# jiangzhengkai/mxdetection

Measured on AMD Instinct MI355X. Metric: images/sec (whole node) Faster R-CNN R50-FPN 3x800x1333, higher is better.
Workload: dtype bf16; 1 GPU; Faster R-CNN ResNet-50-FPN bf16 train step, batch 2/GPU, 3x800x1333 (padded 1344); global_batch=2, parallelism=dp1, frozen=stem+C2, frozen BN folded, optimizer=SGD momentum 0.9 wd 1e-4, launch=hipGraph replay, input=resident, wgrad_side_stream=True, rpn_branch_stream=True, grouped_wgrad=True, filter_prefetch_hints=True, params_trainable=41538304

## Files before the change

### include/mxdet.h

```cpp
#ifndef MXDET_H_
#define MXDET_H_

#include <stddef.h>
#include <stdint.h>

#ifdef __cplusplus
extern "C" {
#endif

#define MXDET_OK 0
#define MXDET_EINVAL (-1)
#define MXDET_ESHAPE (-2)
#define MXDET_EWORKSPACE (-3)
#define MXDET_EHIP (-4)
#define MXDET_ERCCL (-5)

#define MXDET_DTYPE_F32 0
#define MXDET_DTYPE_BF16 1

typedef void* mxdet_stream_t;

const char* mxdet_last_error(void);
const char* mxdet_version(void);

// ... 241 lines not shown
} mxdet_wgrad_item_t;
size_t mxdet_conv2d_wgrad_grouped_table_bytes(int32_t n);
int mxdet_conv2d_wgrad_grouped_plan(const mxdet_wgrad_item_t* items, int32_t n, void* table_host, size_t table_bytes,
                                    size_t* workspace_bytes, int32_t* grid_wgrad, int32_t* grid_big,
                                    int32_t* grid_reduce);
int mxdet_conv2d_wgrad_grouped(const void* table_dev, int32_t n, int32_t grid_wgrad, int32_t grid_big,
                               int32_t grid_reduce, void* workspace, size_t workspace_bytes, size_t workspace_needed,
                               mxdet_stream_t stream);
int mxdet_conv2d_wgrad_grouped_parts(const void* table_dev, int32_t n, int32_t grid_wgrad, int32_t grid_big,
                                     int32_t grid_reduce, int32_t parts, void* workspace, size_t workspace_bytes,
                                     size_t workspace_needed, mxdet_stream_t stream);
int mxdet_filter_transpose(const uint16_t* w, int32_t Cout, int32_t KH, int32_t KW, int32_t Cin,
                           uint16_t* wt, mxdet_stream_t stream);

int mxdet_filter_transpose_batched(const void* descs_dev, int32_t ndesc, int32_t total_tiles,
                                   mxdet_stream_t stream);

#define MXDET_RPN_SPARSE_MAX_LEVELS 8
#define MXDET_RPN_SPARSE_ZERO 1
#define MXDET_RPN_SPARSE_DT 2
#define MXDET_RPN_SPARSE_WGRAD 4
#define MXDET_RPN_SPARSE_DGRAD 8
#define MXDET_RPN_SPARSE_DTMAP 16
typedef struct {
  int32_t num_levels, N, A, C, Ch, smax;
  int32_t H[MXDET_RPN_SPARSE_MAX_LEVELS], W[MXDET_RPN_SPARSE_MAX_LEVELS];
  int32_t accumulate[MXDET_RPN_SPARSE_MAX_LEVELS];
  const void* P[MXDET_RPN_SPARSE_MAX_LEVELS];
  const void* t[MXDET_RPN_SPARSE_MAX_LEVELS];
  const void* tbits[MXDET_RPN_SPARSE_MAX_LEVELS];
  const void* gh[MXDET_RPN_SPARSE_MAX_LEVELS];
  void* dP[MXDET_RPN_SPARSE_MAX_LEVELS];
  void* dt[MXDET_RPN_SPARSE_MAX_LEVELS];
} mxdet_rpn_sparse_t;
int mxdet_rpn_sparse_list(const mxdet_rpn_sparse_t* d, const int32_t* labels, int32_t* list, int32_t* state,
                          int32_t* map, mxdet_stream_t stream);
int mxdet_rpn_sparse_backward(const mxdet_rpn_sparse_t* d, const int32_t* list, const int32_t* state,
                              const int32_t* map, const uint16_t* wt_out, const uint16_t* wt_conv, uint16_t* dts,
                              uint16_t* ghs, float* dw_out, float* db_out, float* dw_conv, float* db_conv,
                              int32_t parts, mxdet_stream_t stream);

typedef struct {
  int32_t N, H, W, C;
  int32_t Ho, Wo;
  int32_t KH, KW;
  int32_t stride, pad;
  int32_t groups;
  int32_t modulated;
  int32_t off_channels;
  int32_t accumulate;
} mxdet_deform_desc_t;
int mxdet_deform_im2col(const mxdet_deform_desc_t* d, const uint16_t* x, const uint16_t* off, uint16_t* col,
                        mxdet_stream_t stream);
int mxdet_deform_col2im_coord(const mxdet_deform_desc_t* d, const uint16_t* x, const uint16_t* off,
                              const uint16_t* dcol, uint16_t* doff, mxdet_stream_t stream);
size_t mxdet_deform_col2im_workspace_bytes(const mxdet_deform_desc_t* d);
int mxdet_deform_col2im(const mxdet_deform_desc_t* d, const uint16_t* off, const uint16_t* dcol, uint16_t* dx,
                        void* workspace, size_t workspace_bytes, mxdet_stream_t stream);

typedef struct {
  int32_t N, HW, C, G;
  float eps;
  int32_t relu;
// ... 81 lines not shown
```

### mxdetection_amd/_lib.py

```python
import ctypes as C
import os

_HERE = os.path.dirname(os.path.abspath(__file__))
LIB_PATH = os.environ.get("MXDET_LIB") or os.path.join(_HERE, "libmxdet_hip.so")

c_i32, c_i64, c_u32, c_f32, c_sz, c_vp = C.c_int32, C.c_int64, C.c_uint32, C.c_float, C.c_size_t, C.c_void_p


class PyramidT(C.Structure):
    _fields_ = [
        ("num_levels", c_i32), ("A", c_i32),
        ("H", c_i32 * 8), ("W", c_i32 * 8), ("stride", c_i32 * 8),
        ("cls", c_vp * 8), ("reg", c_vp * 8),
        ("cls_sn", c_i64 * 8), ("cls_sy", c_i64 * 8), ("cls_sx", c_i64 * 8), ("cls_sa", c_i64 * 8),
        ("reg_sn", c_i64 * 8), ("reg_sy", c_i64 * 8), ("reg_sx", c_i64 * 8), ("reg_sc", c_i64 * 8),
        ("dtype", c_i32), ("classes", c_i32),
        ("base_anchors", c_vp * 8),
    ]


class FeatPyramidT(C.Structure):
    _fields_ = [
        ("num_levels", c_i32), ("lvl_min", c_i32),
        ("H", c_i32 * 8), ("W", c_i32 * 8),
# ... 28 lines not shown

class DeformDescT(C.Structure):
    _fields_ = [
        ("N", c_i32), ("H", c_i32), ("W", c_i32), ("C", c_i32),
        ("Ho", c_i32), ("Wo", c_i32), ("KH", c_i32), ("KW", c_i32),
        ("stride", c_i32), ("pad", c_i32), ("groups", c_i32), ("modulated", c_i32),
        ("off_channels", c_i32), ("accumulate", c_i32),
    ]


class DpoolDescT(C.Structure):
    _fields_ = [
        ("pyr", FeatPyramidT), ("N", c_i32), ("C", c_i32), ("PH", c_i32), ("PW", c_i32),
        ("sample_per_part", c_i32), ("trans_std", c_f32), ("modulated", c_i32),
        ("trans_stride", c_i32), ("mask_stride", c_i32), ("accumulate", c_i32),
    ]


class GnDescT(C.Structure):
    _fields_ = [("N", c_i32), ("HW", c_i32), ("C", c_i32), ("G", c_i32), ("eps", c_f32), ("relu", c_i32),
                ("accumulate", c_i32)]


class RpnSparseT(C.Structure):
    _fields_ = [("num_levels", c_i32), ("N", c_i32), ("A", c_i32), ("C", c_i32), ("Ch", c_i32), ("smax", c_i32),
                ("H", c_i32 * 8), ("W", c_i32 * 8), ("accumulate", c_i32 * 8),
                ("P", c_vp * 8), ("t", c_vp * 8), ("tbits", c_vp * 8), ("gh", c_vp * 8), ("dP", c_vp * 8), ("dt", c_vp * 8)]


WgradItemT._fields_ = [("desc", ConvDescT), ("x", c_vp), ("dy", c_vp), ("dw", c_vp), ("db", c_vp)]
ConvItemT._fields_ = [("desc", ConvDescT), ("src", c_vp), ("filt", c_vp), ("bias", c_vp), ("residual", c_vp),
                      ("relu_mask", c_vp), ("dst", c_vp)]

P = C.POINTER

SIGNATURES = {
    "mxdet_last_error": (C.c_char_p, []),
    "mxdet_version": (C.c_char_p, []),
    "mxdet_box_iou": (c_i32, [c_vp, c_i64, c_vp, c_i64, c_vp, c_vp]),
    "mxdet_generate_anchors": (c_i32, [c_vp, c_i32, c_i32, c_i32, c_i32, c_vp, c_vp]),
    "mxdet_nms_batched_workspace_bytes": (c_sz, [c_i32, c_i32]),
    "mxdet_nms_batched": (c_i32, [c_vp, c_vp, c_vp, c_i32, c_i32, c_f32, c_i32, c_vp, c_vp, c_vp, c_sz, c_vp]),
    "mxdet_soft_nms_batched": (c_i32, [c_vp, c_vp, c_vp, c_i32, c_i32, c_i32, c_f32, c_f32, c_f32, c_i32, c_vp, c_vp, c_vp,
                                       c_vp]),
    "mxdet_pixel_shuffle2_inv_relu": (c_i32, [c_vp, c_vp, c_i64, c_i32, c_i32, c_i32, c_vp, c_vp]),
    "mxdet_mask_paste_workspace_bytes": (c_sz, [c_i64, c_i32]),
    "mxdet_mask_paste": (c_i32, [c_vp, c_vp, c_i64, c_i32, c_i32, c_i32, c_i32, c_f32, c_vp, c_vp, c_sz, c_vp]),
    "mxdet_retina_detect_workspace_bytes": (c_sz, [c_vp, c_i32, c_i32]),
    "mxdet_retina_detect": (c_i32, [c_vp, c_i32, c_vp, c_i32, c_f32, c_f32, c_i32, c_vp, c_vp, c_vp, c_sz, c_vp]),
    "mxdet_retina_detect_soft": (c_i32, [c_vp, c_i32, c_vp, c_i32, c_f32, c_f32, c_i32, c_vp, c_vp, c_vp, c_sz, c_i32, c_f32,
# ... 58 lines not shown
    "mxdet_pixel_shuffle2": (c_i32, [c_vp, c_i64, c_i32, c_i32, c_i32, c_i32, c_vp, c_vp]),
    "mxdet_mask_loss_workspace_bytes": (c_sz, [c_i64, c_i32]),
    "mxdet_mask_loss": (c_i32, [c_vp, c_vp, c_vp, c_i64, c_i32, c_i32, c_f32, c_vp, c_vp, c_vp, c_sz, c_vp]),
    "mxdet_conv2d_fwd": (c_i32, [P(ConvDescT), c_vp, c_vp, c_vp, c_vp, c_vp, c_vp]),
    "mxdet_conv2d_fwd_chain": (c_i32, [P(ConvDescT), c_vp, c_vp, c_vp, c_vp, c_vp, c_i32, c_i32, c_vp, c_vp, c_vp, c_vp, c_i32,
                                       c_i32, c_vp, c_vp]),
    "mxdet_conv2d_fwd_splitk_workspace_bytes": (c_sz, [P(ConvDescT), c_i32]),
    "mxdet_conv2d_fwd_splitk": (c_i32, [P(ConvDescT), c_vp, c_vp, c_vp, c_vp, c_vp, c_i32, c_vp, c_sz, c_vp]),
    "mxdet_conv2d_dgrad": (c_i32, [P(ConvDescT), c_vp, c_vp, c_vp, c_vp, c_vp, c_vp]),
    "mxdet_conv2d_wgrad_workspace_bytes": (c_sz, [P(ConvDescT)]),
    "mxdet_conv2d_wgrad": (c_i32, [P(ConvDescT), c_vp, c_vp, c_vp, c_vp, c_vp, c_sz, c_vp]),
    "mxdet_conv2d_grouped_table_bytes": (c_sz, [c_i32]),
    "mxdet_conv2d_grouped_plan": (c_i32, [P(ConvItemT), c_i32, c_i32, c_vp, c_sz, P(c_i32), P(c_i32)]),
    "mxdet_conv2d_grouped": (c_i32, [c_vp, c_i32, c_i32, c_i32, c_i32, c_vp]),
    "mxdet_conv2d_wgrad_grouped_table_bytes": (c_sz, [c_i32]),
    "mxdet_conv2d_wgrad_grouped_plan": (c_i32, [P(WgradItemT), c_i32, c_vp, c_sz, P(c_sz), P(c_i32), P(c_i32), P(c_i32)]),
    "mxdet_conv2d_wgrad_grouped": (c_i32, [c_vp, c_i32, c_i32, c_i32, c_i32, c_vp, c_sz, c_sz, c_vp]),
    "mxdet_conv2d_wgrad_grouped_parts": (c_i32, [c_vp, c_i32, c_i32, c_i32, c_i32, c_i32, c_vp, c_sz, c_sz, c_vp]),
    "mxdet_debug_force_conv_cfg": (c_i32, [c_i32]),
    "mxdet_debug_force_wgrad_ksplit": (c_i32, [c_i32]),
    "mxdet_rpn_sparse_list": (c_i32, [P(RpnSparseT), c_vp, c_vp, c_vp, c_vp, c_vp]),
    "mxdet_rpn_sparse_backward": (c_i32, [P(RpnSparseT), c_vp, c_vp, c_vp, c_vp, c_vp, c_vp, c_vp, c_vp, c_vp, c_vp, c_vp,
                                          c_i32, c_vp]),
    "mxdet_filter_transpose": (c_i32, [c_vp, c_i32, c_i32, c_i32, c_i32, c_vp, c_vp]),
    "mxdet_filter_transpose_batched": (c_i32, [c_vp, c_i32, c_i32, c_vp]),
    "mxdet_deform_im2col": (c_i32, [P(DeformDescT), c_vp, c_vp, c_vp, c_vp]),
    "mxdet_deform_col2im_coord": (c_i32, [P(DeformDescT), c_vp, c_vp, c_vp, c_vp, c_vp]),
    "mxdet_deform_col2im_workspace_bytes": (c_sz, [P(DeformDescT)]),
    "mxdet_deform_col2im": (c_i32, [P(DeformDescT), c_vp, c_vp, c_vp, c_vp, c_sz, c_vp]),
    "mxdet_dpool_fwd": (c_i32, [P(DpoolDescT), c_vp, c_vp, c_i64, c_vp, c_vp, c_vp, c_vp]),
    "mxdet_dpool_bwd_trans": (c_i32, [P(DpoolDescT), c_vp, c_vp, c_i64, c_vp, c_vp, c_vp, c_vp, c_vp, c_vp]),
    "mxdet_dpool_bwd_feat_workspace_bytes": (c_sz, [P(DpoolDescT), c_i64]),
    "mxdet_dpool_bwd_feat": (c_i32, [P(DpoolDescT), c_vp, c_vp, c_i64, c_vp, c_vp, c_vp, c_vp, c_sz, c_vp]),
    "mxdet_group_norm_workspace_bytes": (c_sz, [P(GnDescT), c_i32]),
    "mxdet_group_norm_fwd": (c_i32, [P(GnDescT), c_vp, c_vp, c_vp, c_vp, c_vp, c_vp, c_vp, c_sz, c_vp]),
    "mxdet_group_norm_bwd": (c_i32, [P(GnDescT), c_vp, c_vp, c_vp, c_vp, c_vp, c_vp, c_vp, c_vp, c_vp, c_vp, c_vp, c_sz,
                                     c_vp]),
    "mxdet_debug_group_norm_route": (c_i32, [P(GnDescT)]),
    "mxdet_stem_conv7x7": (c_i32, [c_vp, c_i32, c_i32, c_i32, c_i32, c_vp, c_vp, c_vp, c_vp]),
    "mxdet_stem_conv7x7_pool": (c_i32, [c_vp, c_i32, c_i32, c_i32, c_i32, c_vp, c_vp, c_vp, c_vp]),
    "mxdet_maxpool3x3s2": (c_i32, [c_vp, c_i32, c_i32, c_i32, c_i32, c_vp, c_vp]),
    "mxdet_subsample2": (c_i32, [c_vp, c_i32, c_i32, c_i32, c_i32, c_vp, c_vp]),
    "mxdet_subsample2_bwd": (c_i32, [c_vp, c_i32, c_i32, c_i32, c_i32, c_i32, c_vp, c_vp]),
    "mxdet_upsample2_bwd": (c_i32, [c_vp, c_i32, c_i32, c_i32, c_i32, c_i32, c_vp, c_vp]),
    "mxdet_add_bf16": (c_i32, [c_vp, c_vp, c_i64, c_vp, c_vp]),
    "mxdet_relu_bwd_bf16": (c_i32, [c_vp, c_vp, c_i64, c_vp, c_vp]),
# ... 73 lines not shown
```

### mxdetection_amd/csrc/rpn_sparse.hip

```cpp
#include "common.h"

namespace mxdet {

constexpr int kSpLevels = MXDET_RPN_SPARSE_MAX_LEVELS;
constexpr int kSpMaxSlots = 8192;

struct SpGeo {
  int L, N, A, C, Ch, smax, CT;
  int H[kSpLevels], W[kSpLevels], coff[kSpLevels + 1];
  const uint16_t* P[kSpLevels];
  const uint16_t* t[kSpLevels];
  const unsigned char* tbits[kSpLevels];
  const uint16_t* gh[kSpLevels];
  uint16_t* dP[kSpLevels];
  uint16_t* dt[kSpLevels];
  int acc[kSpLevels];
  const int* list;
  const int* state;
  const int* map;
  const uint16_t* wt_out;
  const uint16_t* wt_conv;
  uint16_t* dts;
  uint16_t* ghs;
  float* dw_out;
// ... 240 lines not shown
            const bf16x8_t bw = *(const bf16x8_t*)(wbase + (size_t)j * 16 * K9 + t * g.C + k);
            acc[j] = __builtin_amdgcn_mfma_f32_16x16x32_bf16(a, bw, acc[j], 0, 0, 0);
          }
        }
      }
    }
#pragma unroll
    for (int r = 0; r < 4; ++r) {
      const int row = fq * 4 + r;
      const int rl = __shfl(dl, row), rpix = __shfl(dpix, row);
      if (rpix < 0) continue;
      uint16_t* drow = g.dP[rl] + (size_t)rpix * g.C + cit * 64 + frow;
      const bool accum = g.acc[rl] != 0;
#pragma unroll
      for (int j = 0; j < 4; ++j) {
        float v = acc[j][r] + 0.0f;
        if (accum) v += bf16_bits_to_f32(drow[j * 16]);
        drow[j * 16] = sp_bf16(v);
      }
    }
  }
}

static int sp_zero_levels(const SpGeo& g, uint16_t* const* ptr, const int* skip, hipStream_t s) {
  for (int l = 0; l < g.L;) {
    if (skip && skip[l]) { ++l; continue; }
    MXDET_REQUIRE(ptr[l] != nullptr && ((uintptr_t)ptr[l] & 15) == 0, MXDET_EINVAL, "rpn_sparse_backward: level %d null / unaligned", l);
    char* p0 = (char*)ptr[l];
    char* p1 = p0;
    while (l < g.L && !(skip && skip[l]) && (char*)ptr[l] == p1) {
      p1 += (size_t)g.N * g.H[l] * g.W[l] * g.C * 2;
      ++l;
    }
    const long long n16 = (long long)(p1 - p0) / 16;
    hipLaunchKernelGGL(rpn_sparse_zero_kernel, dim3((unsigned)ceil_div<long long>(n16, 256)), dim3(256), 0, s, (uint4*)p0, n16);
  }
  return MXDET_OK;
}

static int sp_fill(SpGeo& g, const mxdet_rpn_sparse_t* d, const char* who) {
  MXDET_REQUIRE(d != nullptr, MXDET_EINVAL, "%s: null descriptor", who);
  MXDET_REQUIRE(d->num_levels > 0 && d->num_levels <= kSpLevels && d->N > 0 && d->A > 0, MXDET_ESHAPE,
                "%s: 1..%d levels, N > 0, A > 0", who, kSpLevels);
  MXDET_REQUIRE(d->C > 0 && d->C % 64 == 0 && d->Ch == 64, MXDET_ESHAPE, "%s: C %d must be a multiple of 64 and Ch %d must be 64",
                who, d->C, d->Ch);
  MXDET_REQUIRE(d->smax > 0 && d->smax <= kSpMaxSlots, MXDET_ESHAPE, "%s: smax %d must be in 1..%d", who, d->smax, kSpMaxSlots);
// ... 57 lines not shown
    for (int l = 0; l < g.L; ++l) g.dt[l] = (uint16_t*)d->dt[l];
    rc = sp_zero_levels(g, g.dt, nullptr, s);
    if (rc) return rc;
  }
  if (parts & MXDET_RPN_SPARSE_DT) {
    MXDET_REQUIRE(wt_out, MXDET_EINVAL, "rpn_sparse_backward: null wt_out");
    for (int l = 0; l < g.L; ++l)
      MXDET_REQUIRE(g.gh[l] && (g.tbits[l] || g.t[l]), MXDET_EINVAL, "rpn_sparse_backward: level %d: null gh / mask", l);
    hipLaunchKernelGGL(rpn_sparse_dt_kernel, dim3((unsigned)ceil_div(g.smax, 16)), dim3(64), 0, s, g);
  }
  if (parts & MXDET_RPN_SPARSE_WGRAD) {
    MXDET_REQUIRE(dw_out && db_out && dw_conv && db_conv, MXDET_EINVAL, "rpn_sparse_backward: null weight-gradient pointer");
    for (int l = 0; l < g.L; ++l)
      MXDET_REQUIRE(g.P[l] && g.t[l], MXDET_EINVAL, "rpn_sparse_backward: level %d: null P / t", l);
    const int ct = g.C / 64;
    hipLaunchKernelGGL(rpn_sparse_wgrad_kernel, dim3((unsigned)(9 * ct * ct + ct)), dim3(256), 0, s, g);
  }
  if (parts & MXDET_RPN_SPARSE_DGRAD) {
    MXDET_REQUIRE(wt_conv, MXDET_EINVAL, "rpn_sparse_backward: null wt_conv");
    for (int l = 0; l < g.L; ++l)
      MXDET_REQUIRE(g.dP[l], MXDET_EINVAL, "rpn_sparse_backward: level %d: null dP", l);
    hipLaunchKernelGGL(rpn_sparse_dgrad_kernel, dim3((unsigned)ceil_div(9 * g.smax, 16)), dim3(256), 0, s, g);
  }
  return check_launch("rpn_sparse_backward");
}
```

### mxdetection_amd/models/rpn_heads/rpn_head.py

```python
import os

import torch

from ...core import anchor as A_
from ...core import loss as L_
from ...ops import dense
from ...ops.proposal import PyramidProposal
from ...ops import rpn_sparse as RS
from ...ops.rpn_sparse import MAX_SLOTS, RPNSparse
from ..utils.layers import ConvLayer, cached_buf

HEAD_CPAD = 64


RELU_BITS = os.environ.get("MXDET_TUNE_RELU_BITS", "1") == "1"
RPN_SPARSE = int(os.environ.get("MXDET_TUNE_RPN_SPARSE", "1"))


class RPNHead:
    def __init__(self, channels, strides, arena, ws, device, gen, ratios=(0.5, 1.0, 2.0), scales=(8,),
                 pre_nms_top_n=2000, post_nms_top_n=2000, nms_thresh=0.7, min_size=0.0, batch_size=256,
                 fg_fraction=0.5, fg_thresh=0.7, bg_thresh=0.3, sigma=3.0, seed=99):
        kw = dict(arena=arena, ws=ws, device=device, gen=gen)
        self.A = len(ratios) * len(scales)
        assert 5 * self.A <= HEAD_CPAD
        self.out = ConvLayer("rpn.out", channels, HEAD_CPAD, 1, init_std=0.01, cout_real=5 * self.A, **kw)
        self.conv = ConvLayer("rpn.conv", channels, channels, 3, init_std=0.01, **kw)
        self.strides = list(strides)
        self.base = [torch.from_numpy(A_.generate_base_anchors(s, ratios, scales)).to(device) for s in strides]
        self.proposal = PyramidProposal(self.base, strides, pre_nms_top_n, post_nms_top_n, nms_thresh, min_size)
        self.batch_size, self.fg_fraction, self.fg_thresh, self.bg_thresh = batch_size, fg_fraction, fg_thresh, bg_thresh
        self.sigma, self.seed, self.device, self.C = sigma, seed, device, channels
        self.bufs = {}
        self.anchors = None
        self.level_shapes = None

    def layers(self):
        return [self.out, self.conv]

# ... 83 lines not shown
        grouped = self.out.ws.grouping
        for l in range(L):
            self.out.backward_weight(self.t[l], self.gh[l], accumulate=(l > 0) and not grouped)
        self.out.backward_data(self.gh[0], self.t[0].shape, relu_mask=self.t[0], out=dt[0], relu_bits=self.tbits[0])
        dense.conv2d_group("dgrad", [self.out.dgrad_call(self.gh[l], self.t[l].shape, relu_mask=self.t[l], out=dt[l],
                                                         relu_bits=self.tbits[l])
                                     for l in range(1, L)], self.device)
        for l in range(L):
            self.conv.backward_weight(self.P[l], dt[l], accumulate=(l > 0) and not grouped)
        self.conv.backward_data(dt[0], self.P[0].shape, accumulate=dP_has_grad[0], out=dP[0])
        dense.conv2d_group("dgrad", [self.conv.dgrad_call(dt[l], self.P[l].shape, accumulate=dP_has_grad[l], out=dP[l])
                                     for l in range(1, L)], self.device)
        if flush:
            self.out.ws.flush()

    def _backward_sparse(self, dP, dP_has_grad, flush=True):
        g = self.out.arena
        grads = (g.view(self.out.wi, "g"), g.view(self.out.bi, "g"), g.view(self.conv.wi, "g"), g.view(self.conv.bi, "g"))
        if self.sparse_wgrad:
            self.sparse.backward(self.P, self.t, self.tbits, self.gh, dP, dP_has_grad, self.out.wt, self.conv.wt, *grads)
            return
        L = len(self.h)
        grouped = self.out.ws.grouping
        for l in range(L):
            self.out.backward_weight(self.t[l], self.gh[l], accumulate=(l > 0) and not grouped)
        self.sparse.backward(self.P, self.t, self.tbits, self.gh, dP, dP_has_grad, self.out.wt, self.conv.wt, *grads,
                             parts=RS.ZERO | RS.DT | RS.DTMAP | RS.DGRAD, dt=self.dt_map)
        for l in range(L):
            self.conv.backward_weight(self.P[l], self.dt_map[l], accumulate=(l > 0) and not grouped)
        if flush:
            self.out.ws.flush()
```

### mxdetection_amd/ops/dense.py

```python
import ctypes as C

import torch

from .. import _lib
from .._lib import ConvDescT, check, ptr, stream_ptr

_DT = {torch.float32: 0, torch.bfloat16: 1}


def mem_range(*tensors):
    spans = [(t.data_ptr(), t.numel() * t.element_size()) for t in tensors]
    bases = {t.untyped_storage().data_ptr() for t in tensors}
    if len(bases) == 1:
        lo = min(p for p, _ in spans)
        hi = max(p + n for p, n in spans)
        if hi - lo <= 2 * sum(n for _, n in set(spans)):
            return (lo, hi - lo)
    return spans[0]


def conv_desc(N, H, W, Cin, Cout, KH, KW, stride, pad, relu=False, res_upsample=False, accumulate=False, prefetch=None,
              relu_bits=None):
    d = ConvDescT()
    if relu_bits is not None:
# ... 140 lines not shown
    key = (kind,) + tuple(tuple(t.data_ptr() if torch.is_tensor(t) else t for t in c) for c in calls)
    if PF_TRACE is not None and calls:
        PF_TRACE.append((None, "g", mem_range(*[c[1] for c in calls]), key if len(calls) > 1 else None))
    if len(calls) == 1:
        plan = None
    else:
        plan = _group_plans.get(key)
        if plan is None and not torch.cuda.is_current_stream_capturing():
            plan = GroupedConv(kind, calls, device, GROUP_HINTS.get(key))
            _group_plans[key] = plan
    if plan is not None:
        plan.launch()
        return
    for c in calls:
        if kind == "fwd":
            x, w, bias, residual, stride, pad, relu, res_up, out = c[:9]
            conv2d_forward(x, w, bias, residual, stride, pad, relu, res_up, out, bits_out=c[9] if len(c) > 9 else None)
        else:
            dy, wt, x_shape, KH, KW, stride, pad, residual, relu_mask, accumulate, out = c[:11]
            conv2d_dgrad(dy, wt, x_shape, KH, KW, stride, pad, residual, relu_mask, accumulate, out,
                         relu_bits=c[11] if len(c) > 11 else None)


class GroupedWgrad:

    def __init__(self, calls, device):
        lib = _lib.load()
        n = len(calls)
        items = (_lib.WgradItemT * n)()
        self.keep = calls
        self.flops = 0.0
        self.heaviest = (0.0, "")
        for it, (x, dy, KH, KW, stride, pad, dw, db, accumulate) in zip(items, calls):
            N, H, W, Cin = x.shape
            it.desc = conv_desc(N, H, W, Cin, dy.shape[3], KH, KW, stride, pad, accumulate=accumulate)
            it.x, it.dy, it.dw, it.db = x.data_ptr(), dy.data_ptr(), dw.data_ptr(), (db.data_ptr() if db is not None else None)
            fl = 2.0 * dy.shape[0] * dy.shape[1] * dy.shape[2] * dy.shape[3] * KH * KW * Cin
            self.flops += fl
            if fl > self.heaviest[0]:
                self.heaviest = (fl, "N=%d %dx%d %d->%d %dx%d" % (N, H, W, Cin, dy.shape[3], KH, KW))
        nbytes = lib.mxdet_conv2d_wgrad_grouped_table_bytes(n)
        host = (C.c_ubyte * nbytes)()
        ws, gw, gb, gr = C.c_size_t(0), C.c_int32(0), C.c_int32(0), C.c_int32(0)
        check(lib.mxdet_conv2d_wgrad_grouped_plan(items, n, host, nbytes, C.byref(ws), C.byref(gw), C.byref(gb),
                                                  C.byref(gr)), "conv2d_wgrad_grouped_plan")
        self.grid_big = gb.value
        self.table = torch.frombuffer(bytearray(host), dtype=torch.uint8).clone().to(device)
        self.n, self.grid_wgrad, self.grid_reduce, self.workspace_bytes = n, gw.value, gr.value, ws.value

    def launch(self, workspace):
        check(_lib.load().mxdet_conv2d_wgrad_grouped(ptr(self.table), self.n, self.grid_wgrad, self.grid_big, self.grid_reduce,
                                                     ptr(workspace), workspace.numel() if workspace is not None else 0,
                                                     self.workspace_bytes, stream_ptr()), "conv2d_wgrad_grouped")


def filter_transpose(w, out=None):
    lib = _lib.load()
    Cout, KH, KW, Cin = w.shape
    if out is None:
        out = torch.empty((Cin, KH, KW, Cout), dtype=torch.bfloat16, device=w.device)
    check(lib.mxdet_filter_transpose(ptr(w), Cout, KH, KW, Cin, ptr(out), stream_ptr()), "filter_transpose")
    return out


def make_transpose_table(pairs, device):
    import struct
    buf = bytearray()
    tile0 = 0
    for w, wt in pairs:
        Cout, KH, KW, Cin = w.shape
        buf += struct.pack("<QQiiii", w.data_ptr(), wt.data_ptr(), Cout, KH * KW, Cin, tile0)
# ... 150 lines not shown
```

### mxdetection_amd/ops/rpn_sparse.py

```python
import ctypes as C

import torch

from .. import _lib
from .._lib import RpnSparseT, check, ptr, stream_ptr

ZERO, DT, WGRAD, DGRAD, DTMAP = 1, 2, 4, 8, 16
ALL = ZERO | DT | WGRAD | DGRAD
MAX_SLOTS = 8192


class RPNSparse:

    def __init__(self, level_shapes, N, A, C_, Ch, smax, device):
        self.level_shapes, self.N, self.A, self.C, self.Ch, self.smax = list(level_shapes), N, A, C_, Ch, smax
        self.CT = sum(h * w for h, w in level_shapes)
        i32 = dict(dtype=torch.int32, device=device)
        self.list = torch.full((2 * smax,), -1, **i32)
        self.state = torch.zeros((2,), **i32)
        self.map = torch.full((N * self.CT,), -1, **i32)
        self.dts = torch.zeros((smax, C_), dtype=torch.bfloat16, device=device)
        self.ghs = torch.zeros((smax, Ch), dtype=torch.bfloat16, device=device)
        self._descs = {}

    def _desc(self, P=None, t=None, tbits=None, gh=None, dP=None, accumulate=None, dt=None):
        L = len(self.level_shapes)
        ops = (P, t, tbits, gh, dP, dt)
        key = tuple(None if o is None else tuple(0 if x is None else x.data_ptr() for x in o) for o in ops)
        key += (None if accumulate is None else tuple(bool(a) for a in accumulate),)
        d = self._descs.get(key)
        if d is None:
            d = RpnSparseT()
            d.num_levels, d.N, d.A, d.C, d.Ch, d.smax = L, self.N, self.A, self.C, self.Ch, self.smax
            for l, (h, w) in enumerate(self.level_shapes):
                d.H[l], d.W[l] = h, w
                d.accumulate[l] = int(bool(accumulate[l])) if accumulate is not None else 0
                for name, o in zip(("P", "t", "tbits", "gh", "dP", "dt"), ops):
                    if o is not None and o[l] is not None:
                        getattr(d, name)[l] = o[l].data_ptr()
            self._descs[key] = d
        return d

    def build_list(self, labels):
        assert labels.dtype == torch.int32 and labels.numel() == self.N * self.CT * self.A and labels.is_contiguous()
        check(_lib.load().mxdet_rpn_sparse_list(C.byref(self._desc()), ptr(labels), ptr(self.list), ptr(self.state),
                                                ptr(self.map), stream_ptr()), "rpn_sparse_list")

    def backward(self, P, t, tbits, gh, dP, accumulate, wt_out, wt_conv, dw_out, db_out, dw_conv, db_conv, parts=ALL, dt=None):
        d = self._desc(P, t, tbits, gh, dP, accumulate, dt)
        check(_lib.load().mxdet_rpn_sparse_backward(C.byref(d), ptr(self.list), ptr(self.state), ptr(self.map), ptr(wt_out),
                                                    ptr(wt_conv), ptr(self.dts), ptr(self.ghs), ptr(dw_out), ptr(db_out),
                                                    ptr(dw_conv), ptr(db_conv), parts, stream_ptr()), "rpn_sparse_backward")
```

Before: 452.6 images/sec.

## Add ordered sparse RPN weight-gradient kernel replacing dense grouped wgrad for head

```diff
diff --git a/include/mxdet.h b/include/mxdet.h
--- a/include/mxdet.h
+++ b/include/mxdet.h
@@ -287,6 +287,17 @@
 #define MXDET_RPN_SPARSE_WGRAD 4
 #define MXDET_RPN_SPARSE_DGRAD 8
 #define MXDET_RPN_SPARSE_DTMAP 16
+#define MXDET_RPN_SPARSE_WGRAD_ORDERED 32
+#define MXDET_RPN_ORDERED_WORK_INTS(smax) (10 * (smax) + 32)
+typedef struct {
+  int32_t kind;
+  int32_t H, W;
+  int32_t halves_per_slab;
+  int32_t slab0;
+  int32_t fold_ksplit;
+  int32_t bias_pixels;
+  int32_t bias_splits;
+} mxdet_rpn_ordered_item_t;
 typedef struct {
   int32_t num_levels, N, A, C, Ch, smax;
   int32_t H[MXDET_RPN_SPARSE_MAX_LEVELS], W[MXDET_RPN_SPARSE_MAX_LEVELS];
@@ -297,6 +308,8 @@
   const void* gh[MXDET_RPN_SPARSE_MAX_LEVELS];
   void* dP[MXDET_RPN_SPARSE_MAX_LEVELS];
   void* dt[MXDET_RPN_SPARSE_MAX_LEVELS];
+  const mxdet_rpn_ordered_item_t* ordered;
+  void* ordered_work;
 } mxdet_rpn_sparse_t;
 int mxdet_rpn_sparse_list(const mxdet_rpn_sparse_t* d, const int32_t* labels, int32_t* list, int32_t* state,
                           int32_t* map, mxdet_stream_t stream);
@@ -304,6 +317,7 @@
                               const int32_t* map, const uint16_t* wt_out, const uint16_t* wt_conv, uint16_t* dts,
                               uint16_t* ghs, float* dw_out, float* db_out, float* dw_conv, float* db_conv,
                               int32_t parts, mxdet_stream_t stream);
+int mxdet_rpn_ordered_schedule(const void* table_host, int32_t n, int32_t num_levels, mxdet_rpn_ordered_item_t* items);
 
 typedef struct {
   int32_t N, H, W, C;
diff --git a/mxdetection_amd/_lib.py b/mxdetection_amd/_lib.py
--- a/mxdetection_amd/_lib.py
+++ b/mxdetection_amd/_lib.py
@@ -74,10 +74,16 @@
                 ("accumulate", c_i32)]
 
 
+class RpnOrderedItemT(C.Structure):
+    _fields_ = [("kind", c_i32), ("H", c_i32), ("W", c_i32), ("halves_per_slab", c_i32), ("slab0", c_i32),
+                ("fold_ksplit", c_i32), ("bias_pixels", c_i32), ("bias_splits", c_i32)]
+
+
 class RpnSparseT(C.Structure):
     _fields_ = [("num_levels", c_i32), ("N", c_i32), ("A", c_i32), ("C", c_i32), ("Ch", c_i32), ("smax", c_i32),
                 ("H", c_i32 * 8), ("W", c_i32 * 8), ("accumulate", c_i32 * 8),
-                ("P", c_vp * 8), ("t", c_vp * 8), ("tbits", c_vp * 8), ("gh", c_vp * 8), ("dP", c_vp * 8), ("dt", c_vp * 8)]
+                ("P", c_vp * 8), ("t", c_vp * 8), ("tbits", c_vp * 8), ("gh", c_vp * 8), ("dP", c_vp * 8), ("dt", c_vp * 8),
+                ("ordered", C.POINTER(RpnOrderedItemT)), ("ordered_work", c_vp)]
 
 
 WgradItemT._fields_ = [("desc", ConvDescT), ("x", c_vp), ("dy", c_vp), ("dw", c_vp), ("db", c_vp)]
@@ -182,6 +188,7 @@
     "mxdet_rpn_sparse_list": (c_i32, [P(RpnSparseT), c_vp, c_vp, c_vp, c_vp, c_vp]),
     "mxdet_rpn_sparse_backward": (c_i32, [P(RpnSparseT), c_vp, c_vp, c_vp, c_vp, c_vp, c_vp, c_vp, c_vp, c_vp, c_vp, c_vp,
                                           c_i32, c_vp]),
+    "mxdet_rpn_ordered_schedule": (c_i32, [c_vp, c_i32, c_i32, P(RpnOrderedItemT)]),
     "mxdet_filter_transpose": (c_i32, [c_vp, c_i32, c_i32, c_i32, c_i32, c_vp, c_vp]),
     "mxdet_filter_transpose_batched": (c_i32, [c_vp, c_i32, c_i32, c_vp]),
     "mxdet_deform_im2col": (c_i32, [P(DeformDescT), c_vp, c_vp, c_vp, c_vp]),
diff --git a/mxdetection_amd/csrc/rpn_sparse.hip b/mxdetection_amd/csrc/rpn_sparse.hip
--- a/mxdetection_amd/csrc/rpn_sparse.hip
+++ b/mxdetection_amd/csrc/rpn_sparse.hip
@@ -1,4 +1,5 @@
 #include "common.h"
+#include "wgrad3_tile.h"
 
 namespace mxdet {
 
@@ -286,6 +287,260 @@
   }
 }
 
+struct SpOrd {
+  int kind[2][kSpLevels];
+  int hps[2][kSpLevels];
+  int bpix[2][kSpLevels];
+  int* work;
+};
+constexpr int kOrdNewHalf = 1, kOrdNewSlab = 2, kOrdNewBias = 4;
+constexpr int kOrdHalves = 8;
+constexpr int kOrdImg = 32 * 128;
+
+__device__ __forceinline__ int4* sp_ord_ent(const SpGeo& g, const SpOrd& o, int q) { return (int4*)(o.work + 16) + (size_t)q * g.smax; }
+__device__ __forceinline__ int* sp_ord_hsf(const SpGeo& g, const SpOrd& o, int q) {
+  return o.work + 16 + 8 * (size_t)g.smax + (size_t)q * (g.smax + 1);
+}
+
+__global__ void __launch_bounds__(1024) rpn_sparse_order_kernel(const SpGeo g, const SpOrd o) {
+  __shared__ int keys[kSpMaxSlots];
+  __shared__ unsigned short ordv[kSpMaxSlots];
+  __shared__ __attribute__((aligned(16))) unsigned char nhalf[2][kSpMaxSlots];
+  const int tid = threadIdx.x;
+  const int S = g.state[0];
+  for (int i = tid; i < S; i += 1024) {
+    const SpCell c = sp_decode(g, g.list[i]);
+    keys[i] = g.N * g.coff[c.l] + c.pix;
+  }
+  __syncthreads();
+  for (int i = tid; i < S; i += 1024) {
+    const int k = keys[i];
+    int rank = 0;
+    for (int j = 0; j < S; ++j) rank += keys[j] < k ? 1 : 0;
+    ordv[rank] = (unsigned short)i;
+  }
+  __syncthreads();
+  for (int r = tid; r < S; r += 1024) {
+    const int s = ordv[r];
+    const SpCell c = sp_decode(g, g.list[s]);
+    SpCell cp = c;
+    if (r > 0) cp = sp_decode(g, g.list[ordv[r - 1]]);
+    const int H = g.H[c.l], W = g.W[c.l], Hp = g.H[cp.l], Wp = g.W[cp.l];
+#pragma unroll
+    for (int q = 0; q < 2; ++q) {
+      const int v = o.kind[q][c.l] ? (c.n * H + c.h) * (W + 1) + c.w : c.pix;
+      const int vp = o.kind[q][cp.l] ? (cp.n * Hp + cp.h) * (Wp + 1) + cp.w : cp.pix;
+      const int hs = v >> 5, hsp = vp >> 5;
+      const bool first = r == 0 || cp.l != c.l;
+      int fl = 0;
+      if (first || hsp != hs) fl |= kOrdNewHalf;
+      if (first || hsp / o.hps[q][cp.l] != hs / o.hps[q][c.l]) fl |= kOrdNewSlab;
+      if (first || cp.pix / o.bpix[q][cp.l] != c.pix / o.bpix[q][c.l]) fl |= kOrdNewBias;
+      nhalf[q][r] = (unsigned char)(fl & kOrdNewHalf);
+      sp_ord_ent(g, o, q)[r] = make_int4(s | (c.l << 16), c.pix, c.h | (c.w << 16), (v & 31) | (fl << 5));
+    }
+  }
+  __syncthreads();
+  for (int r = tid; r < S; r += 1024) {
+#pragma unroll
+    for (int q = 0; q < 2; ++q) {
+      const unsigned* w32 = (const unsigned*)nhalf[q];
+      int cnt = 0;
+      const int words = (r + 1) >> 2;
+      for (int j = 0; j < words; ++j) cnt += __popc(w32[j]);
+      for (int j = words * 4; j <= r; ++j) cnt += nhalf[q][j];
+      int* wq = (int*)&sp_ord_ent(g, o, q)[r];
+      wq[3] |= (cnt - 1) << 8;
+      int* hsf = sp_ord_hsf(g, o, q);
+      if (nhalf[q][r]) hsf[cnt - 1] = r;
+      if (r == S - 1) { o.work[q] = cnt; hsf[cnt] = S; }
+    }
+  }
+  if (S == 0 && tid < 2) { o.work[tid] = 0; sp_ord_hsf(g, o, tid)[0] = 0; }
+}
+
+__device__ __forceinline__ int sp_ord_g2(int row) { return ((row >> 1) & 1) | (((row >> 3) & 1) << 1); }
+
+__global__ void __launch_bounds__(256) rpn_sparse_wgrad_ordered_kernel(const SpGeo g, const SpOrd o) {
+  __shared__ __attribute__((aligned(1024))) unsigned char img[2 * kOrdHalves * 2 * kOrdImg];
+  __shared__ int rb[kSpMaxSlots / kOrdHalves + 2];
+  __shared__ int rflag[2][kOrdHalves];
+  const int tid = threadIdx.x, lane = tid & 63, frow = lane & 15, fq = lane >> 4;
+  const int wid = __builtin_amdgcn_readfirstlane(tid >> 6);
+  const int ct = g.C / 64;
+  const int nconv = 9 * ct * ct;
+  const int S = g.state[0];
+  int b = blockIdx.x;
+  if (b >= nconv + ct) {
+    b -= nconv + ct;
+    const int nb_conv = g.C / 16;
+    const int q = b < nb_conv ? 1 : 0;
+    const int c0 = (q ? b : b - nb_conv) * 16;
+    const uint16_t* X = q ? g.dts : g.ghs;
+    const int ldx = q ? g.C : g.Ch;
+    float* db = q ? g.db_conv : g.db_out;
+    const int4* ent = sp_ord_ent(g, o, q);
+    uint16_t* xv = (uint16_t*)img;
+    int* xm = (int*)(img + 256 * 32);
+    const int c = tid >> 4, r0 = tid & 15;
+    float part = 0.0f, fold = 0.0f;
+    for (int e0 = 0; e0 < S; e0 += 256) {
+      __syncthreads();
+      if (e0 + tid < S) {
+        const int4 en = ent[e0 + tid];
+        const uint16_t* row = X + (size_t)(en.x & 0xffff) * ldx + c0;
+        *(uint4*)(xv + tid * 16) = *(const uint4*)row;
+        *(uint4*)(xv + tid * 16 + 8) = *(const uint4*)(row + 8);
+        xm[tid] = (en.y & 15) | (((en.w >> 5) & kOrdNewBias) ? (1 << 31) : 0);
+      }
+      __syncthreads();
+      const int n = S - e0 < 256 ? S - e0 : 256;
+      for (int i = 0; i < n; ++i) {
+        const int m = xm[i];
+        if (m < 0) {
+          float t = __shfl(part, lane & 48);
+          for (int r = 1; r < 16; ++r) t += __shfl(part, (lane & 48) + r);
+          fold += t;
+          part = 0.0f;
+        }
+        if ((m & 15) == r0) part += bf16_bits_to_f32(xv[i * 16 + c]);
+      }
+    }
+    float t = __shfl(part, lane & 48);
+    for (int r = 1; r < 16; ++r) t += __shfl(part, (lane & 48) + r);
+    fold += t;
+    if (r0 == 0) db[c0 + c] = fold;
+    return;
+  }
+  const bool conv = b < nconv;
+  const int q = conv ? 1 : 0;
+  const uint16_t* X;
+  int ldx, x0, y0, dh, dw, ldw;
+  float* out;
+  if (conv) {
+    const int tap = b / (ct * ct), r = b - tap * ct * ct, cot = r / ct, cit = r - cot * ct;
+    X = g.dts; ldx = g.C; x0 = cot * 64; y0 = cit * 64; dh = tap / 3 - 1; dw = tap % 3 - 1;
+    ldw = 9 * g.C;
+    out = g.dw_conv + (size_t)x0 * ldw + tap * g.C + y0;
+  } else {
+    b -= nconv;
+    X = g.ghs; ldx = g.Ch; x0 = 0; y0 = b * 64; dh = 0; dw = 0;
+    ldw = g.C;
+    out = g.dw_out + y0;
+  }
+  const int4* ent = sp_ord_ent(g, o, q);
+  const int* hsf = sp_ord_hsf(g, o, q);
+  const int nh = o.work[q];
+  const int nr = (nh + kOrdHalves - 1) / kOrdHalves;
+  for (int i = tid; i <= nr; i += 256) rb[i] = hsf[i * kOrdHalves < nh ? i * kOrdHalves : nh];
+  for (int i = tid; i < (int)sizeof(img) / 16; i += 256) ((uint4*)img)[i] = make_uint4(0u, 0u, 0u, 0u);
+  __syncthreads();
+  const int eidx = tid >> 4, op = (tid >> 3) & 1, c8 = tid & 7;
+  auto locate = [&](const int4& en, int rd) -> int {
+    const int k = en.w & 31, hi = (en.w >> 8) - rd * kOrdHalves;
+    return (((rd & 1) * kOrdHalves + hi) * 2 + op) * kOrdImg + k * 128 + ((((c8 >> 1) ^ sp_ord_g2(k))) << 5) + ((c8 & 1) << 4);
+  };
+  auto fetch = [&](const int4& en) -> uint4 {
+    if (op == 0) return *(const uint4*)(X + (size_t)(en.x & 0xffff) * ldx + x0 + c8 * 8);
+    const int l = en.x >> 16, hh = (en.z & 0xffff) + dh, ww = (en.z >> 16) + dw;
+    const uint16_t* y = conv ? g.P[l] : g.t[l];
+    if (hh < 0 || hh >= g.H[l] || ww < 0 || ww >= g.W[l]) return make_uint4(0u, 0u, 0u, 0u);
+    return *(const uint4*)(y + (size_t)(en.y + dh * g.W[l] + dw) * g.C + y0 + c8 * 8);
+  };
+  auto flag = [&](const int4& en, int rd) {
+    if (op == 0 && c8 == 0 && ((en.w >> 5) & kOrdNewHalf))
+      rflag[rd & 1][(en.w >> 8) - rd * kOrdHalves] = (en.w >> 5) & kOrdNewSlab;
+  };
+  const int4 none = make_int4(-1, 0, 0, 0);
+  auto load_ent = [&](int rd, int4 (&en)[2]) {
+#pragma unroll
+    for (int p = 0; p < 2; ++p) {
+      en[p] = none;
+      if (rd < nr) {
+        const int e = rb[rd] + p * 16 + eidx;
+        if (e < rb[rd + 1]) en[p] = ent[e];
+      }
+    }
+  };
+  struct Stage { int4 enw[2]; uint4 dat[2]; int woff[2]; };
+  int4 en[2];
+  Stage st0, st1;
+  auto load_dat = [&](int rd, Stage& st) {
+#pragma unroll
+    for (int p = 0; p < 2; ++p) {
+      st.enw[p] = en[p];
+      st.woff[p] = -1;
+      if (en[p].x >= 0) { st.woff[p] = locate(en[p], rd); st.dat[p] = fetch(en[p]); }
+    }
+  };
+  f32x4_t acc[4], fold[4];
+#pragma unroll
+  for (int j = 0; j < 4; ++j) { acc[j] = f32x4_t{0.f, 0.f, 0.f, 0.f}; fold[j] = acc[j]; }
+  const int qq = (lane >> 2) & 3, pp = lane & 3;
+  const int rowa = 8 * fq + qq, g2a = sp_ord_g2(rowa);
+  const int offa = rowa * 128 + ((wid ^ g2a) << 5) + pp * 8;
+  int offb[4];
+#pragma unroll
+  for (int j = 0; j < 4; ++j) offb[j] = kOrdImg + rowa * 128 + ((j ^ g2a) << 5) + pp * 8;
+  typedef __attribute__((ext_vector_type(8))) short s16x8_t;
+  auto frag = [&](const unsigned char* base, int off) -> bf16x8_t {
+    const s16x4_t lo = tr_read(base, off), hi = tr_read(base, off + 512);
+    return __builtin_bit_cast(bf16x8_t, (s16x8_t){lo[0], lo[1], lo[2], lo[3], hi[0], hi[1], hi[2], hi[3]});
+  };
+  load_ent(0, en);
+  load_dat(0, st0);
+  load_ent(1, en);
+  load_dat(1, st1);
+  load_ent(2, en);
+  for (int rd = 0; rd < nr; ++rd) {
+    const int e0 = rb[rd], e1 = rb[rd + 1];
+    int zoff[2];
+#pragma unroll
+    for (int p = 0; p < 2; ++p) {
+      zoff[p] = st0.woff[p];
+      if (st0.woff[p] >= 0) { *(uint4*)(img + st0.woff[p]) = st0.dat[p]; flag(st0.enw[p], rd); }
+    }
+    for (int e = e0 + 32 + eidx; e < e1; e += 16) {
+      const int4 x = ent[e];
+      *(uint4*)(img + locate(x, rd)) = fetch(x);
+      flag(x, rd);
+    }
+    __syncthreads();
+    st0 = st1;
+    load_dat(rd + 2, st1);
+    load_ent(rd + 3, en);
+    const unsigned char* set = img + (rd & 1) * kOrdHalves * 2 * kOrdImg;
+    const int nhere = nh - rd * kOrdHalves < kOrdHalves ? nh - rd * kOrdHalves : kOrdHalves;
+    int fl[kOrdHalves];
+#pragma unroll
+    for (int hh = 0; hh < kOrdHalves; ++hh) fl[hh] = rflag[rd & 1][hh];
+#pragma unroll
+    for (int hh = 0; hh < kOrdHalves; ++hh) {
+      if (hh >= nhere) break;
+      const unsigned char* base = set + hh * 2 * kOrdImg;
+      if (__builtin_amdgcn_readfirstlane(fl[hh])) {
+#pragma unroll
+        for (int j = 0; j < 4; ++j) { fold[j] += acc[j]; acc[j] = f32x4_t{0.f, 0.f, 0.f, 0.f}; }
+      }
+      const bf16x8_t a = frag(base, offa);
+#pragma unroll
+      for (int j = 0; j < 4; ++j) acc[j] = __builtin_amdgcn_mfma_f32_16x16x32_bf16(a, frag(base, offb[j]), acc[j], 0, 0, 0);
+    }
+    __syncthreads();
+#pragma unroll
+    for (int p = 0; p < 2; ++p)
+      if (zoff[p] >= 0) *(uint4*)(img + zoff[p]) = make_uint4(0u, 0u, 0u, 0u);
+    for (int e = e0 + 32 + eidx; e < e1; e += 16) *(uint4*)(img + locate(ent[e], rd)) = make_uint4(0u, 0u, 0u, 0u);
+  }
+#pragma unroll
+  for (int j = 0; j < 4; ++j) fold[j] += acc[j];
+#pragma unroll
+  for (int j = 0; j < 4; ++j)
+#pragma unroll
+    for (int r = 0; r < 4; ++r)
+      out[(size_t)(wid * 16 + fq * 4 + r) * ldw + j * 16 + frow] = fold[j][r];
+}
+
 static int sp_zero_levels(const SpGeo& g, uint16_t* const* ptr, const int* skip, hipStream_t s) {
   for (int l = 0; l < g.L;) {
     if (skip && skip[l]) { ++l; continue; }
@@ -389,5 +644,68 @@
       MXDET_REQUIRE(g.dP[l], MXDET_EINVAL, "rpn_sparse_backward: level %d: null dP", l);
     hipLaunchKernelGGL(rpn_sparse_dgrad_kernel, dim3((unsigned)ceil_div(9 * g.smax, 16)), dim3(256), 0, s, g);
   }
+  if (parts & MXDET_RPN_SPARSE_WGRAD_ORDERED) {
+    MXDET_REQUIRE(!(parts & MXDET_RPN_SPARSE_WGRAD), MXDET_EINVAL, "rpn_sparse_backward: WGRAD and WGRAD_ORDERED write the same gradients");
+    MXDET_REQUIRE(dw_out && db_out && dw_conv && db_conv, MXDET_EINVAL, "rpn_sparse_backward: null weight-gradient pointer");
+    MXDET_REQUIRE(d->ordered && d->ordered_work && ((uintptr_t)d->ordered_work & 15) == 0, MXDET_EINVAL,
+                  "rpn_sparse_backward: WGRAD_ORDERED needs the schedule and 16-byte aligned scratch");
+    SpOrd o;
+    memset(&o, 0, sizeof(o));
+    o.work = (int*)d->ordered_work;
+    for (int q = 0; q < 2; ++q)
+      for (int l = 0; l < g.L; ++l) {
+        const mxdet_rpn_ordered_item_t& it = d->ordered[q * g.L + l];
+        MXDET_REQUIRE((it.kind == 0 || it.kind == 1) && it.H == g.H[l] && it.W == g.W[l] && it.halves_per_slab > 0 &&
+                          it.bias_pixels > 0 && it.bias_pixels % 16 == 0,
+                      MXDET_EINVAL, "rpn_sparse_backward: schedule record %d does not describe level %d", q * g.L + l, l);
+        MXDET_REQUIRE((long long)g.N * g.H[l] * (g.W[l] + 1) < (1ll << 31), MXDET_ESHAPE, "rpn_sparse_backward: level %d too large", l);
+        const int prev = l == 0 ? -1 : d->ordered[q * g.L + l - 1].slab0;
+        MXDET_REQUIRE((l == 0 ? it.slab0 == 0 : it.slab0 > prev) && it.slab0 < it.fold_ksplit &&
+                          it.fold_ksplit == d->ordered[q * g.L].fold_ksplit && it.bias_splits >= 1,
+                      MXDET_EINVAL, "rpn_sparse_backward: schedule record %d: slabs out of item order", q * g.L + l);
+        o.kind[q][l] = it.kind; o.hps[q][l] = it.halves_per_slab; o.bpix[q][l] = it.bias_pixels;
+      }
+    for (int l = 0; l < g.L; ++l)
+      MXDET_REQUIRE(g.P[l] && g.t[l], MXDET_EINVAL, "rpn_sparse_backward: level %d: null P / t", l);
+    const int ct = g.C / 64;
+    hipLaunchKernelGGL(rpn_sparse_order_kernel, dim3(1), dim3(1024), 0, s, g, o);
+    hipLaunchKernelGGL(rpn_sparse_wgrad_ordered_kernel, dim3((unsigned)(9 * ct * ct + ct + g.C / 16 + g.Ch / 16)), dim3(256), 0, s, g, o);
+  }
   return check_launch("rpn_sparse_backward");
 }
+
+extern "C" int mxdet_rpn_ordered_schedule(const void* table_host, int32_t n, int32_t num_levels, mxdet_rpn_ordered_item_t* items) {
+  clear_error();
+  MXDET_REQUIRE(table_host && items && num_levels > 0 && num_levels <= kSpLevels && n == 2 * num_levels, MXDET_EINVAL,
+                "rpn_ordered_schedule: a table of 2 * num_levels items");
+  const WgradG* t = (const WgradG*)table_host;
+  for (int q = 0; q < 2; ++q) {
+    const WgradG& own = t[q * num_levels];
+    int next = 0;
+    for (int l = 0; l < num_levels; ++l) {
+      const int i = q * num_levels + l;
+      const WgradP& p = t[i].p;
+      MXDET_REQUIRE(p.dw == own.p.dw && p.db == own.p.db && p.db != nullptr && !p.accumulate && t[i].nparams == own.nparams,
+                    MXDET_EINVAL, "rpn_ordered_schedule: item %d is not a level of filter %d (with a bias, no accumulate)", i, q);
+      MXDET_REQUIRE(p.stride == 1 && p.Ho == p.H && p.Wo == p.W && (q ? (p.KH == 3 && p.KW == 3 && p.pad == 1)
+                                                                      : (p.KH == 1 && p.KW == 1 && p.pad == 0)),
+                    MXDET_EINVAL, "rpn_ordered_schedule: item %d is not the head's %s convolution", i, q ? "3x3" : "1x1");
+      const size_t slab_bytes = (size_t)own.nparams * sizeof(float);
+      const size_t doff = (size_t)p.slab - (size_t)own.p.slab, boff = (size_t)p.bslab - (size_t)own.p.bslab;
+      mxdet_rpn_ordered_item_t& it = items[i];
+      it.kind = p.t3_nwg > 0 ? 1 : 0;
+      it.H = p.H; it.W = p.W;
+      it.halves_per_slab = it.kind ? p.t3_steps * (kT3Px / 32) : p.steps_per_split * (kWgradBKP / 32);
+      it.slab0 = (int32_t)(doff / slab_bytes);
+      it.fold_ksplit = own.fold_ksplit;
+      it.bias_pixels = p.steps_per_split * kWgradBKP;
+      it.bias_splits = p.ksplit;
+      MXDET_REQUIRE(doff % slab_bytes == 0 && it.slab0 == next && boff == (size_t)next * p.Cout * sizeof(float), MXDET_EINVAL,
+                    "rpn_ordered_schedule: item %d: its slabs do not follow item %d's", i, i - 1);
+      next += it.kind ? p.t3_ksplit : p.ksplit;
+    }
+    MXDET_REQUIRE(next == own.fold_ksplit, MXDET_EINVAL, "rpn_ordered_schedule: filter %d folds %d slabs, its levels write %d", q,
+                  own.fold_ksplit, next);
+  }
+  return MXDET_OK;
+}
diff --git a/mxdetection_amd/models/rpn_heads/rpn_head.py b/mxdetection_amd/models/rpn_heads/rpn_head.py
--- a/mxdetection_amd/models/rpn_heads/rpn_head.py
+++ b/mxdetection_amd/models/rpn_heads/rpn_head.py
@@ -15,6 +15,7 @@
 
 RELU_BITS = os.environ.get("MXDET_TUNE_RELU_BITS", "1") == "1"
 RPN_SPARSE = int(os.environ.get("MXDET_TUNE_RPN_SPARSE", "1"))
+RPN_ORDERED = int(os.environ.get("MXDET_TUNE_RPN_ORDERED", "1"))
 
 
 class RPNHead:
@@ -144,6 +145,15 @@
             return
         L = len(self.h)
         grouped = self.out.ws.grouping
+        if grouped and RPN_ORDERED and self.out.train_bias and self.conv.train_bias:
+            if self.sparse.ordered is None and not torch.cuda.is_current_stream_capturing():
+                self.sparse.plan_ordered(
+                    [(self.t[l], self.gh[l], 1, 1, 1, 0, grads[0], grads[1], False) for l in range(L)] +
+                    [(self.P[l], self.dt_map[l], 3, 3, 1, 1, grads[2], grads[3], False) for l in range(L)])
+            if self.sparse.ordered is not None:
+                self.sparse.backward(self.P, self.t, self.tbits, self.gh, dP, dP_has_grad, self.out.wt, self.conv.wt, *grads,
+                                     parts=RS.ZERO | RS.DT | RS.DGRAD | RS.WGRAD_ORDERED)
+                return
         for l in range(L):
             self.out.backward_weight(self.t[l], self.gh[l], accumulate=(l > 0) and not grouped)
         self.sparse.backward(self.P, self.t, self.tbits, self.gh, dP, dP_has_grad, self.out.wt, self.conv.wt, *grads,
diff --git a/mxdetection_amd/ops/dense.py b/mxdetection_amd/ops/dense.py
--- a/mxdetection_amd/ops/dense.py
+++ b/mxdetection_amd/ops/dense.py
@@ -186,31 +186,38 @@
                          relu_bits=c[11] if len(c) > 11 else None)
 
 
+def plan_wgrad_group(calls):
+    lib = _lib.load()
+    n = len(calls)
+    items = (_lib.WgradItemT * n)()
+    for it, (x, dy, KH, KW, stride, pad, dw, db, accumulate) in zip(items, calls):
+        N, H, W, Cin = x.shape
+        it.desc = conv_desc(N, H, W, Cin, dy.shape[3], KH, KW, stride, pad, accumulate=accumulate)
+        it.x, it.dy, it.dw, it.db = x.data_ptr(), dy.data_ptr(), dw.data_ptr(), (db.data_ptr() if db is not None else None)
+    nbytes = lib.mxdet_conv2d_wgrad_grouped_table_bytes(n)
+    host = (C.c_ubyte * nbytes)()
+    ws, gw, gb, gr = C.c_size_t(0), C.c_int32(0), C.c_int32(0), C.c_int32(0)
+    check(lib.mxdet_conv2d_wgrad_grouped_plan(items, n, host, nbytes, C.byref(ws), C.byref(gw), C.byref(gb),
+                                              C.byref(gr)), "conv2d_wgrad_grouped_plan")
+    return host, ws.value, gw.value, gb.value, gr.value
+
+
 class GroupedWgrad:
 
     def __init__(self, calls, device):
-        lib = _lib.load()
-        n = len(calls)
-        items = (_lib.WgradItemT * n)()
         self.keep = calls
         self.flops = 0.0
         self.heaviest = (0.0, "")
-        for it, (x, dy, KH, KW, stride, pad, dw, db, accumulate) in zip(items, calls):
+        for x, dy, KH, KW, stride, pad, dw, db, accumulate in calls:
             N, H, W, Cin = x.shape
-            it.desc = conv_desc(N, H, W, Cin, dy.shape[3], KH, KW, stride, pad, accumulate=accumulate)
-            it.x, it.dy, it.dw, it.db = x.data_ptr(), dy.data_ptr(), dw.data_ptr(), (db.data_ptr() if db is not None else None)
             fl = 2.0 * dy.shape[0] * dy.shape[1] * dy.shape[2] * dy.shape[3] * KH * KW * Cin
             self.flops += fl
             if fl > self.heaviest[0]:
                 self.heaviest = (fl, "N=%d %dx%d %d->%d %dx%d" % (N, H, W, Cin, dy.shape[3], KH, KW))
-        nbytes = lib.mxdet_conv2d_wgrad_grouped_table_bytes(n)
-        host = (C.c_ubyte * nbytes)()
-        ws, gw, gb, gr = C.c_size_t(0), C.c_int32(0), C.c_int32(0), C.c_int32(0)
-        check(lib.mxdet_conv2d_wgrad_grouped_plan(items, n, host, nbytes, C.byref(ws), C.byref(gw), C.byref(gb),
-                                                  C.byref(gr)), "conv2d_wgrad_grouped_plan")
-        self.grid_big = gb.value
+        host, ws, gw, gb, gr = plan_wgrad_group(calls)
+        self.grid_big = gb
         self.table = torch.frombuffer(bytearray(host), dtype=torch.uint8).clone().to(device)
-        self.n, self.grid_wgrad, self.grid_reduce, self.workspace_bytes = n, gw.value, gr.value, ws.value
+        self.n, self.grid_wgrad, self.grid_reduce, self.workspace_bytes = len(calls), gw, gr, ws
 
     def launch(self, workspace):
         check(_lib.load().mxdet_conv2d_wgrad_grouped(ptr(self.table), self.n, self.grid_wgrad, self.grid_big, self.grid_reduce,
diff --git a/mxdetection_amd/ops/rpn_sparse.py b/mxdetection_amd/ops/rpn_sparse.py
--- a/mxdetection_amd/ops/rpn_sparse.py
+++ b/mxdetection_amd/ops/rpn_sparse.py
@@ -3,9 +3,10 @@
 import torch
 
 from .. import _lib
-from .._lib import RpnSparseT, check, ptr, stream_ptr
+from .._lib import RpnOrderedItemT, RpnSparseT, check, ptr, stream_ptr
+from . import dense
 
-ZERO, DT, WGRAD, DGRAD, DTMAP = 1, 2, 4, 8, 16
+ZERO, DT, WGRAD, DGRAD, DTMAP, WGRAD_ORDERED = 1, 2, 4, 8, 16, 32
 ALL = ZERO | DT | WGRAD | DGRAD
 MAX_SLOTS = 8192
 
@@ -21,6 +22,18 @@
         self.map = torch.full((N * self.CT,), -1, **i32)
         self.dts = torch.zeros((smax, C_), dtype=torch.bfloat16, device=device)
         self.ghs = torch.zeros((smax, Ch), dtype=torch.bfloat16, device=device)
+        self._descs = {}
+        self.ordered = None
+        self.ordered_work = None
+
+    def plan_ordered(self, calls):
+        L = len(self.level_shapes)
+        assert len(calls) == 2 * L
+        host = dense.plan_wgrad_group(calls)[0]
+        sched = (RpnOrderedItemT * (2 * L))()
+        check(_lib.load().mxdet_rpn_ordered_schedule(host, 2 * L, L, sched), "rpn_ordered_schedule")
+        self.ordered = sched
+        self.ordered_work = torch.zeros((10 * self.smax + 32,), dtype=torch.int32, device=self.list.device)
         self._descs = {}
 
     def _desc(self, P=None, t=None, tbits=None, gh=None, dP=None, accumulate=None, dt=None):
@@ -38,6 +51,9 @@
                 for name, o in zip(("P", "t", "tbits", "gh", "dP", "dt"), ops):
                     if o is not None and o[l] is not None:
                         getattr(d, name)[l] = o[l].data_ptr()
+            if self.ordered is not None:
+                d.ordered = self.ordered
+                d.ordered_work = self.ordered_work.data_ptr()
             self._descs[key] = d
         return d
 
```

After: 465.7 images/sec, median of 6. 2.9% higher.
